# zzzxxxttt/SimpleDepthEstimation

Measured on AMD Instinct MI355X. Metric: training images/sec at 192x640 bs=12/GPU, higher is better.
Workload: dtype bf16; 1 GPU; Supervised ResNet-50 (BASELINE configs[1]), bf16 storage / fp32 accumulate, bs=12/GPU, 192x640, fwd+bwd+optimizer, random-init weights; global_batch=12, parallelism=dp1, hip_graph=True, allreduce_overlap=False

## Files before the change

simpledepthestimation_amd/csrc/conv.hip:

```cpp
#include <type_traits>

#include "common.h"
#include "sde_hip.h"
#include "conv_common.h"

namespace {
using namespace sdeconv;

template <int I> using IC = std::integral_constant<int, I>;

typedef __attribute__((ext_vector_type(4))) float f32x4;
typedef __attribute__((ext_vector_type(8))) __bf16 bf16x8;
typedef __attribute__((ext_vector_type(4))) short s16x4;
typedef __attribute__((ext_vector_type(8))) short s16x8;

template <typename T> struct VecOf;
template <> struct VecOf<float> { static constexpr int V = 4; };
template <> struct VecOf<bf16_t> { static constexpr int V = 8; };
template <> struct VecOf<half_t> { static constexpr int V = 8; };

template <typename T>
__device__ __forceinline__ uint4 gather16(const Gather& g, int n, int ih, int iw, int ci) {
    uint4 z = {0u, 0u, 0u, 0u};
    if (g.reflect) { ih = reflect1(ih, g.IH); iw = reflect1(iw, g.IW); }
// ... 90 lines not shown
    constexpr int CPT = 8 / TPR;
    constexpr int B_ROWS_PER_PASS = NTHREADS / 8;
    constexpr int B_PASSES = (BN + B_ROWS_PER_PASS - 1) / B_ROWS_PER_PASS;
    constexpr int CPAD = 4;
    static_assert(WM * WN == 4, "4 waves");
    extern __shared__ __attribute__((aligned(16))) unsigned char smem[];
    unsigned char* sA = smem;
    unsigned char* sB = smem + 2 * BM * KSTAGE_BYTES;

    const Gather& g = p.g;
    const int tid = threadIdx.x, lane = tid & 63, wave = tid >> 6;
    const int wm = wave / WN, wn = wave % WN;
    const int tiles_n = (p.ldy + BN - 1) / BN;
    const int logical_all = xcd_remap(blockIdx.x, gridDim.x);
    const int tiles_all = gridDim.x / p.ksplit;
    const int split = logical_all / tiles_all, logical = logical_all - split * tiles_all;
    const int tile_m = logical / tiles_n, tile_n = logical - tile_m * tiles_n;
    const int m0 = tile_m * BM, n0 = tile_n * BN;

    const int arow = tid / TPR, ac0 = (tid % TPR) * CPT;
    int an = -1, aih = 0, aiw = 0;
    {
        const int m = m0 + arow;
        if (m < g.M) {
            an = m / (g.OH * g.OW);
            const int rem = m - an * (g.OH * g.OW);
            const int oh = rem / g.OW, ow = rem - oh * g.OW;
            aih = oh * g.stride - g.pad; aiw = ow * g.stride - g.pad;
        }
    }
    const int nk_total = (g.Ktot + BK - 1) / BK;
    const int nk_per = (nk_total + p.ksplit - 1) / p.ksplit;
    const int s_begin = split * nk_per;
    int aci, akh, akw;
    {
        const int k = s_begin * BK + ac0 * V;
        const int tap = k / g.Cin;
        aci = k - tap * g.Cin; akh = tap / g.KW; akw = tap - akh * g.KW;
    }
    const int cc = tid & 7, r0 = tid >> 3;
    const int nk = max(0, min(nk_total, s_begin + nk_per) - s_begin);
    const __amdgpu_buffer_rsrc_t rs0 = make_rsrc(g.x0, (long)g.Bn * g.H0 * g.W0 * g.C0 * (long)sizeof(T));
    const __amdgpu_buffer_rsrc_t rs1 = make_rsrc(g.x1 ? g.x1 : g.x0, g.x1 ? (long)g.Bn * g.IH * g.IW * g.C1 * (long)sizeof(T) : 0);
    const __amdgpu_buffer_rsrc_t rsw = make_rsrc(p.w, (long)p.Cout * g.Ktot * (long)sizeof(T));
    const int mode = src_mode<SRC>(g);
    unsigned rowoff = kOOB;
    if (SRC == SRC_1X1 && an >= 0) rowoff = (unsigned)(((an * g.H0 + aih) * g.W0 + aiw) * g.C0) * (unsigned)sizeof(T);

    const bool kfull = SRC == SRC_1X1 && (g.Ktot % BK) == 0 && !p.no_kfull;
    const bool kfullB = (g.Ktot % BK) == 0 && !p.no_kfull;
    unsigned voffA = kOOB, voffB[B_PASSES];
    if (SRC == SRC_1X1 && an >= 0) voffA = rowoff + (unsigned)(ac0 * V) * (unsigned)sizeof(T);
#pragma unroll
    for (int i = 0; i < B_PASSES; ++i) {
        const int row = r0 + i * B_ROWS_PER_PASS, n = n0 + row;
        voffB[i] = (row < BN && n < p.Cout) ? (unsigned)(n * g.Ktot + cc * V) * (unsigned)sizeof(T) : kOOB;
    }

    uint4 ra[3][CPT], rb[3][B_PASSES];

    auto load_stage = [&](int s, auto SET) {
        constexpr int st = decltype(SET)::value;
        if (SRC == SRC_1X1 && kfull) {
            const unsigned soff = (unsigned)(s_begin + s) * (unsigned)KSTAGE_BYTES;
#pragma unroll
            for (int c = 0; c < CPT; ++c) ra[st][c] = buf_load16s(rs0, voffA + 16u * c, soff);
#pragma unroll
            for (int i = 0; i < B_PASSES; ++i) rb[st][i] = buf_load16s(rsw, voffB[i], soff);
            return;
        }
        if (SRC == SRC_1X1) {
            const int k = (s_begin + s) * BK + ac0 * V;
#pragma unroll
            for (int c = 0; c < CPT; ++c)
                ra[st][c] = buf_load16(rs0, (k + c * V < g.Ktot) ? rowoff + (unsigned)(k + c * V) * (unsigned)sizeof(T) : kOOB);
        } else if (ONE_TAP) {
            unsigned o0, o1;
            gather_off<T, SRC>(g, an >= 0 && akh < g.KH, an, aih + akh, aiw + akw, aci, o0, o1);
#pragma unroll
            for (int c = 0; c < CPT; ++c) {
                uint4 v = buf_load16(rs0, o0 + 16u * c);
                if (mode == SDE_SRC_UPCAT) {
                    const uint4 u = buf_load16(rs1, o1 + 16u * c);
                    v.x |= u.x; v.y |= u.y; v.z |= u.z; v.w |= u.w;
                }
                ra[st][c] = v;
            }
        } else {
            int ci = aci, kh = akh, kw = akw;
#pragma unroll
            for (int c = 0; c < CPT; ++c) {
                unsigned o0, o1;
                gather_off<T, SRC>(g, an >= 0 && kh < g.KH, an, aih + kh, aiw + kw, ci, o0, o1);
                uint4 v = buf_load16(rs0, o0);
                if (mode == SDE_SRC_UPCAT) {
                    const uint4 u = buf_load16(rs1, o1);
                    v.x |= u.x; v.y |= u.y; v.z |= u.z; v.w |= u.w;
                }
                ra[st][c] = v;
                ci += V;
                if (ci == g.Cin) { ci = 0; if (++kw == g.KW) { kw = 0; ++kh; } }
            }
        }
        if (SRC != SRC_1X1) {
            aci += BK;
            while (aci >= g.Cin) { aci -= g.Cin; if (++akw == g.KW) { akw = 0; ++akh; } }
        }
        if (kfullB) {
            const unsigned soff = (unsigned)(s_begin + s) * (unsigned)KSTAGE_BYTES;
#pragma unroll
            for (int i = 0; i < B_PASSES; ++i) rb[st][i] = buf_load16s(rsw, voffB[i], soff);
            return;
        }
        const int k = (s_begin + s) * BK + cc * V;
        const bool kok = k < g.Ktot;
#pragma unroll
        for (int i = 0; i < B_PASSES; ++i) {
            const int row = r0 + i * B_ROWS_PER_PASS;
            const int n = n0 + row;
            constexpr bool rows_fit = B_ROWS_PER_PASS * B_PASSES <= BN;
            const unsigned ow = (kok && (rows_fit || row < BN) && n < p.Cout) ? (unsigned)(n * g.Ktot + k) * (unsigned)sizeof(T) : kOOB;
            rb[st][i] = buf_load16(rsw, ow);
        }
    };
    auto store_stage = [&](int buf, auto SET) {
        constexpr int st = decltype(SET)::value;
#pragma unroll
        for (int c = 0; c < CPT; ++c)
            *reinterpret_cast<uint4*>(sA + (size_t)(buf * BM + arow) * KSTAGE_BYTES + (((ac0 + c) ^ (arow & 7)) << 4)) = ra[st][c];
#pragma unroll
        for (int i = 0; i < B_PASSES; ++i) {
            const int row = r0 + i * B_ROWS_PER_PASS;
            if (B_ROWS_PER_PASS * B_PASSES <= BN || row < BN)
                *reinterpret_cast<uint4*>(sB + (size_t)(buf * BN + row) * KSTAGE_BYTES + ((cc ^ (row & 7)) << 4)) = rb[st][i];
        }
    };

    f32x4 acc[FM][FN];
#pragma unroll
    for (int i = 0; i < FM; ++i)
#pragma unroll
        for (int j = 0; j < FN; ++j) acc[i][j] = f32x4{0.f, 0.f, 0.f, 0.f};

    const int fr = lane & 15, fg = lane >> 4;
    auto compute_stage = [&](int buf) {
#pragma unroll
        for (int kk = 0; kk < 2; ++kk) {
            uint4 a[FM], b[FN];
            const int ch = kk * 4 + fg;
#pragma unroll
            for (int i = 0; i < FM; ++i) {
                const int row = wm * WTM + i * 16 + fr;
                a[i] = *reinterpret_cast<const uint4*>(sA + (size_t)(buf * BM + row) * KSTAGE_BYTES + ((ch ^ (row & 7)) << 4));
            }
#pragma unroll
            for (int j = 0; j < FN; ++j) {
                const int row = wn * WTN + j * 16 + fr;
                b[j] = *reinterpret_cast<const uint4*>(sB + (size_t)(buf * BN + row) * KSTAGE_BYTES + ((ch ^ (row & 7)) << 4));
            }
#pragma unroll
            for (int i = 0; i < FM; ++i)
#pragma unroll
                for (int j = 0; j < FN; ++j) acc[i][j] = mma64<T>(a[i], b[j], acc[i][j]);
        }
    };
    auto step = [&](int st, auto CUR, auto NXT) {
        if (st >= nk) return;
        if (st + 3 < nk) load_stage(st + 3, CUR);
        compute_stage(st & 1);
        if (st + 1 < nk) store_stage((st + 1) & 1, NXT);
        __syncthreads();
    };
    if (nk > 0) load_stage(0, IC<0>{});
    if (nk > 1) load_stage(1, IC<1>{});
    if (nk > 2) load_stage(2, IC<2>{});
    if (nk > 0) store_stage(0, IC<0>{});
    __syncthreads();
    for (int s = 0; s < nk; s += 3) {
        step(s, IC<0>{}, IC<1>{});
        step(s + 1, IC<1>{}, IC<2>{});
        step(s + 2, IC<2>{}, IC<0>{});
    }

    float* sC = reinterpret_cast<float*>(smem);
#pragma unroll
    for (int i = 0; i < FM; ++i)
#pragma unroll
        for (int j = 0; j < FN; ++j)
#pragma unroll
            for (int r = 0; r < 4; ++r) {
                const int row = wm * WTM + i * 16 + fg * 4 + r, col = wn * WTN + j * 16 + fr;
                sC[row * (BN + CPAD) + col] = acc[i][j][r];
            }
    __syncthreads();
    constexpr int G4 = BN / 4;
    const bool vec_ok = (p.ldy % 4) == 0;
    if (p.ksplit > 1) {
        float* wsp = p.ws + (size_t)split * g.M * p.ldy;
        for (int id = tid; id < BM * G4; id += NTHREADS) {
            const int row = id / G4, c0 = (id - row * G4) * 4;
            const int m = m0 + row, n = n0 + c0;
            if (m >= g.M || n >= p.ldy) continue;
            *reinterpret_cast<float4*>(wsp + (size_t)m * p.ldy + n) = *reinterpret_cast<const float4*>(&sC[row * (BN + CPAD) + c0]);
        }
        return;
    }
    for (int id = tid; id < BM * G4; id += NTHREADS) {
        const int row = id / G4, c0 = (id - row * G4) * 4;
        const int m = m0 + row, n = n0 + c0;
        if (m >= g.M || n >= p.ldy) continue;
        const float4 q = *reinterpret_cast<const float4*>(&sC[row * (BN + CPAD) + c0]);
        float v[4] = {q.x, q.y, q.z, q.w};
#pragma unroll
        for (int e = 0; e < 4; ++e) {
            float t = v[e];
            if (p.bias && n + e < p.Cout) t += p.bias[n + e];
            if (p.act == SDE_ACT_ELU) t = t > 0.f ? t : expm1f(t);
            if (n + e >= p.Cout) t = 0.f;
            v[e] = t;
        }
        T* dst = (T*)p.y + (size_t)m * p.ldy + n;
        T o[4];
#pragma unroll
        for (int e = 0; e < 4; ++e) o[e] = from_f32<T>(v[e]);
        if (vec_ok && n + 4 <= p.ldy) {
            if (sizeof(T) == 2) *reinterpret_cast<uint2*>(dst) = *reinterpret_cast<uint2*>(o);
            else *reinterpret_cast<uint4*>(dst) = *reinterpret_cast<uint4*>(o);
        } else {
            for (int e = 0; e < 4 && n + e < p.ldy; ++e) dst[e] = o[e];
        }
        if (p.stats)
            *reinterpret_cast<float4*>(&sC[row * (BN + CPAD) + c0]) = make_float4(to_f32<T>(o[0]), to_f32<T>(o[1]), to_f32<T>(o[2]), to_f32<T>(o[3]));
    }
    if (p.stats) {
        __syncthreads();
        constexpr int PARTS = NTHREADS / BN >= 1 ? NTHREADS / BN : 1;
        float* red = sC + BM * (BN + CPAD);
        const int c = tid % BN, part = tid / BN;
        const int rows = min(BM, g.M - m0);
        float s1 = 0.f, s2 = 0.f;
        if (part < PARTS)
            for (int r = part; r < rows; r += PARTS) { const float t = sC[r * (BN + CPAD) + c]; s1 += t; s2 += t * t; }
        if (part < PARTS) { red[(part * BN + c) * 2] = s1; red[(part * BN + c) * 2 + 1] = s2; }
        __syncthreads();
        if (tid < BN && n0 + tid < p.Cout) {
            float a = 0.f, b = 0.f;
#pragma unroll
            for (int q = 0; q < PARTS; ++q) { a += red[(q * BN + tid) * 2]; b += red[(q * BN + tid) * 2 + 1]; }
            p.stats[((size_t)tile_m * p.Cout + n0 + tid) * 2 + 0] = a;
            p.stats[((size_t)tile_m * p.Cout + n0 + tid) * 2 + 1] = b;
        }
    }
}

template <typename T>
__global__ void __launch_bounds__(256) splitk_finish_kernel(const float* __restrict__ ws, int S, int M, int ldy, int Cout, const float* __restrict__ bias,
                                                            int act, T* __restrict__ y, float* __restrict__ stats) {
    __shared__ float red[16][64][2];
    const int tiles_n = (ldy + 63) / 64;
    const int tile_m = blockIdx.x / tiles_n, tile_n = blockIdx.x - tile_m * tiles_n;
    const int c0 = tile_n * 64 + (threadIdx.x & 15) * 4, rg = threadIdx.x >> 4;
    float s1[4] = {0.f, 0.f, 0.f, 0.f}, s2[4] = {0.f, 0.f, 0.f, 0.f};
    if (c0 < ldy) {
#pragma unroll
        for (int i = 0; i < 4; ++i) {
            const int m = tile_m * 64 + rg + 16 * i;
            if (m >= M) continue;
            float4 a = *reinterpret_cast<const float4*>(ws + (size_t)m * ldy + c0);
            for (int sp = 1; sp < S; ++sp) {
                const float4 b = *reinterpret_cast<const float4*>(ws + ((size_t)sp * M + m) * ldy + c0);
                a.x += b.x; a.y += b.y; a.z += b.z; a.w += b.w;
            }
            float v[4] = {a.x, a.y, a.z, a.w};
            T o[4];
#pragma unroll
            for (int e = 0; e < 4; ++e) {
                float t = v[e];
                if (bias && c0 + e < Cout) t += bias[c0 + e];
                if (act == SDE_ACT_ELU) t = t > 0.f ? t : expm1f(t);
                if (c0 + e >= Cout) t = 0.f;
                o[e] = from_f32<T>(t);
                const float r = to_f32<T>(o[e]);
                s1[e] += r; s2[e] += r * r;
            }
            T* dst = y + (size_t)m * ldy + c0;
            if (sizeof(T) == 2) *reinterpret_cast<uint2*>(dst) = *reinterpret_cast<uint2*>(o);
            else *reinterpret_cast<uint4*>(dst) = *reinterpret_cast<uint4*>(o);
        }
    }
    if (!stats) return;
#pragma unroll
    for (int e = 0; e < 4; ++e) { red[rg][(threadIdx.x & 15) * 4 + e][0] = s1[e]; red[rg][(threadIdx.x & 15) * 4 + e][1] = s2[e]; }
    __syncthreads();
    if (threadIdx.x < 64 && tile_n * 64 + threadIdx.x < Cout) {
        float a = 0.f, b = 0.f;
#pragma unroll
        for (int q = 0; q < 16; ++q) { a += red[q][threadIdx.x][0]; b += red[q][threadIdx.x][1]; }
        stats[((size_t)tile_m * Cout + tile_n * 64 + threadIdx.x) * 2 + 0] = a;
        stats[((size_t)tile_m * Cout + tile_n * 64 + threadIdx.x) * 2 + 1] = b;
    }
}

constexpr int HT_H = 8, HT_W = 16, HALO_W = HT_W + 2, HALO_PIX = (HT_H + 2) * HALO_W;
constexpr int HPIX_STRIDE = 144;
constexpr int HALO_PASSES = (HALO_PIX * 8 + NTHREADS - 1) / NTHREADS;

template <typename T, int SRC>
__device__ __forceinline__ void halo_pix(const Gather& g, bool ok, int n, int ih, int iw, unsigned& p0, unsigned& p1) {
    if (src_reflect<SRC>(g)) { ih = reflect1(ih, g.IH); iw = reflect1(iw, g.IW); ok = ok & ((unsigned)ih < (unsigned)g.IH) & ((unsigned)iw < (unsigned)g.IW); }
    else ok = ok & ((unsigned)ih < (unsigned)g.IH) & ((unsigned)iw < (unsigned)g.IW);
    p1 = kOOB;
    if (src_mode<SRC>(g) == SDE_SRC_UPCAT) {
        p0 = ok ? (unsigned)(((n * g.H0 + (ih >> 1)) * g.W0 + (iw >> 1)) * g.C0) * (unsigned)sizeof(T) : kOOB;
        p1 = (ok && g.C1 > 0) ? (unsigned)(((n * g.IH + ih) * g.IW + iw) * g.C1) * (unsigned)sizeof(T) : kOOB;
    } else {
        p0 = ok ? (unsigned)(((n * g.H0 + ih) * g.W0 + iw) * g.C0) * (unsigned)sizeof(T) : kOOB;
    }
}

template <typename T, int BN, int WM, int WN, int SRC>
__global__ void __launch_bounds__(NTHREADS, 2) halo3_kernel(IGemmP p) {
    constexpr int V = VecOf<T>::V;
    constexpr int BM = HT_H * HT_W;
    constexpr int BK = KSTAGE_BYTES / (int)sizeof(T);
    constexpr int WTM = BM / WM, WTN = BN / WN;
    constexpr int FM = WTM / 16, FN = WTN / 16;
    constexpr int B_ROWS_PER_PASS = NTHREADS / 8;
    constexpr int B_PASSES = (BN + B_ROWS_PER_PASS - 1) / B_ROWS_PER_PASS;
    constexpr int CPAD = 4;
    static_assert(WM * WN == 4 && sizeof(T) == 2, "4 waves, 16-bit storage");
    extern __shared__ __attribute__((aligned(16))) unsigned char smem[];
    unsigned char* sH = smem;
    unsigned char* sB = smem + HALO_PIX * HPIX_STRIDE;

    const Gather& g = p.g;
    const int mode = src_mode<SRC>(g);
    const int tid = threadIdx.x, lane = tid & 63, wave = tid >> 6;
    const int wm = wave / WN, wn = wave % WN;
    const int tiles_n = (p.ldy + BN - 1) / BN, tiles_x = (g.OW + HT_W - 1) / HT_W, tiles_y = (g.OH + HT_H - 1) / HT_H;
    const int logical = xcd_remap(blockIdx.x, gridDim.x);
    const int tile_m = logical / tiles_n, tile_n = logical - tile_m * tiles_n;
    const int img = tile_m / (tiles_x * tiles_y), trem = tile_m - img * (tiles_x * tiles_y);
    const int oy0 = (trem / tiles_x) * HT_H, ox0 = (trem % tiles_x) * HT_W;
    const int n0 = tile_n * BN;
    const __amdgpu_buffer_rsrc_t rs0 = make_rsrc(g.x0, (long)g.Bn * g.H0 * g.W0 * g.C0 * (long)sizeof(T));
    const __amdgpu_buffer_rsrc_t rs1 = make_rsrc(g.x1 ? g.x1 : g.x0, g.x1 ? (long)g.Bn * g.IH * g.IW * g.C1 * (long)sizeof(T) : 0);
    const __amdgpu_buffer_rsrc_t rsw = make_rsrc(p.w, (long)p.Cout * g.Ktot * (long)sizeof(T));

    const int hc = tid & 7;
    unsigned hp0[HALO_PASSES], hp1[HALO_PASSES];
#pragma unroll
    for (int j = 0; j < HALO_PASSES; ++j) {
        const int hp = (tid >> 3) + 32 * j;
        const int hy = hp / HALO_W, hx = hp - hy * HALO_W;
        halo_pix<T, SRC>(g, hp < HALO_PIX, img, oy0 - g.pad + hy, ox0 - g.pad + hx, hp0[j], hp1[j]);
    }
    const int ncb = (g.Cin + BK - 1) / BK;
    const int nst = ncb * 9;
    uint4 rh[HALO_PASSES];
    auto load_halo = [&](int cb) {
        const int ci = cb * BK + hc * V;
#pragma unroll
        for (int j = 0; j < HALO_PASSES; ++j) {
            unsigned o0, o1 = kOOB;
            if (mode == SDE_SRC_UPCAT) {
                o0 = (ci < g.C0 && hp0[j] != kOOB) ? hp0[j] + (unsigned)ci * (unsigned)sizeof(T) : kOOB;
                o1 = (ci >= g.C0 && ci < g.Cin && hp1[j] != kOOB) ? hp1[j] + (unsigned)(ci - g.C0) * (unsigned)sizeof(T) : kOOB;
            } else {
                o0 = (ci < g.Cin && hp0[j] != kOOB) ? hp0[j] + (unsigned)ci * (unsigned)sizeof(T) : kOOB;
            }
            uint4 v = buf_load16(rs0, o0);
            if (mode == SDE_SRC_UPCAT) {
                const uint4 u = buf_load16(rs1, o1);
                v.x |= u.x; v.y |= u.y; v.z |= u.z; v.w |= u.w;
            }
            rh[j] = v;
        }
    };
    auto store_halo = [&]() {
#pragma unroll
        for (int j = 0; j < HALO_PASSES; ++j) {
            const int hp = (tid >> 3) + 32 * j;
            if (hp < HALO_PIX) *reinterpret_cast<uint4*>(sH + hp * HPIX_STRIDE + hc * 16) = rh[j];
        }
    };
    const int cc = tid & 7, r0 = tid >> 3;
    uint4 rb[3][B_PASSES];
    auto load_b = [&](int s, auto SET) {
        constexpr int st = decltype(SET)::value;
        const int cb = s / 9, tap = s - cb * 9;
        const int ci = cb * BK + cc * V;
        const int k = tap * g.Cin + ci;
#pragma unroll
        for (int i = 0; i < B_PASSES; ++i) {
            const int row = r0 + i * B_ROWS_PER_PASS, n = n0 + row;
            rb[st][i] = buf_load16(rsw, (ci < g.Cin && row < BN && n < p.Cout) ? (unsigned)(n * g.Ktot + k) * (unsigned)sizeof(T) : kOOB);
        }
    };
    auto store_b = [&](int buf, auto SET) {
        constexpr int st = decltype(SET)::value;
#pragma unroll
        for (int i = 0; i < B_PASSES; ++i) {
            const int row = r0 + i * B_ROWS_PER_PASS;
            if (B_ROWS_PER_PASS * B_PASSES <= BN || row < BN)
                *reinterpret_cast<uint4*>(sB + (size_t)(buf * BN + row) * KSTAGE_BYTES + ((cc ^ (row & 7)) << 4)) = rb[st][i];
        }
    };

    f32x4 acc[FM][FN];
#pragma unroll
    for (int i = 0; i < FM; ++i)
#pragma unroll
        for (int j = 0; j < FN; ++j) acc[i][j] = f32x4{0.f, 0.f, 0.f, 0.f};

    const int fr = lane & 15, fg = lane >> 4;
    int abase[FM];
#pragma unroll
    for (int i = 0; i < FM; ++i) abase[i] = ((wm * FM + i) * HALO_W + fr) * HPIX_STRIDE + fg * 16;
    auto compute_stage = [&](int buf, int tap) {
        const int toff = ((tap / 3) * HALO_W + (tap % 3)) * HPIX_STRIDE;
#pragma unroll
        for (int kk = 0; kk < 2; ++kk) {
            uint4 a[FM], b[FN];
#pragma unroll
            for (int i = 0; i < FM; ++i) a[i] = *reinterpret_cast<const uint4*>(sH + abase[i] + toff + kk * 64);
#pragma unroll
            for (int j = 0; j < FN; ++j) {
                const int row = wn * WTN + j * 16 + fr;
                b[j] = *reinterpret_cast<const uint4*>(sB + (size_t)(buf * BN + row) * KSTAGE_BYTES + (((kk * 4 + fg) ^ (row & 7)) << 4));
            }
#pragma unroll
            for (int i = 0; i < FM; ++i)
#pragma unroll
                for (int j = 0; j < FN; ++j) acc[i][j] = mma64<T>(a[i], b[j], acc[i][j]);
        }
    };
    auto step = [&](int st, auto CUR, auto NXT) {
        if (st >= nst) return;
        const int cb = st / 9, tap = st - cb * 9;
        if (st + 3 < nst) load_b(st + 3, CUR);
        if (tap == 0 && cb + 1 < ncb) load_halo(cb + 1);
        compute_stage(st & 1, tap);
        if (st + 1 < nst) store_b((st + 1) & 1, NXT);
        __syncthreads();
        if (tap == 8 && cb + 1 < ncb) {
            store_halo();
            __syncthreads();
        }
    };
    load_halo(0);
    load_b(0, IC<0>{});
    if (nst > 1) load_b(1, IC<1>{});
    if (nst > 2) load_b(2, IC<2>{});
    store_halo();
    store_b(0, IC<0>{});
    __syncthreads();
    for (int s = 0; s < nst; s += 3) {
        step(s, IC<0>{}, IC<1>{});
        step(s + 1, IC<1>{}, IC<2>{});
        step(s + 2, IC<2>{}, IC<0>{});
    }

    float* sC = reinterpret_cast<float*>(smem);
#pragma unroll
    for (int i = 0; i < FM; ++i)
#pragma unroll
        for (int j = 0; j < FN; ++j)
#pragma unroll
            for (int r = 0; r < 4; ++r) {
                const int row = wm * WTM + i * 16 + fg * 4 + r, col = wn * WTN + j * 16 + fr;
                sC[row * (BN + CPAD) + col] = acc[i][j][r];
            }
    __syncthreads();
    constexpr int G4 = BN / 4;
    const bool vec_ok = (p.ldy % 4) == 0;
    if (p.bn_y) {
        static_assert(NTHREADS % G4 == 0, "a thread keeps one channel group");
        const int c0 = (tid % G4) * 4, n = n0 + c0;
        const float4 mean = *reinterpret_cast<const float4*>(p.bnp + n), rstd = *reinterpret_cast<const float4*>(p.bnp + p.Cout + n);
        const float4 scl = *reinterpret_cast<const float4*>(p.bnp + 2 * p.Cout + n), shf = *reinterpret_cast<const float4*>(p.bnp + 3 * p.Cout + n);
        const float mn[4] = {mean.x, mean.y, mean.z, mean.w}, rs[4] = {rstd.x, rstd.y, rstd.z, rstd.w};
        const float sc[4] = {scl.x, scl.y, scl.z, scl.w}, sf[4] = {shf.x, shf.y, shf.z, shf.w};
        float a1[4] = {0.f, 0.f, 0.f, 0.f}, a2[4] = {0.f, 0.f, 0.f, 0.f};
        for (int id = tid; id < BM * G4; id += NTHREADS) {
            const int row = id / G4;
            const int oy = oy0 + row / HT_W, ox = ox0 + row % HT_W;
            if (!(oy < g.OH && ox < g.OW)) continue;
            const size_t off = ((size_t)(img * g.OH + oy) * g.OW + ox) * p.ldy + n;
            const uint2 yr = *reinterpret_cast<const uint2*>((const T*)p.bn_y + off);
            const T* yt = reinterpret_cast<const T*>(&yr);
            const float4 q = *reinterpret_cast<const float4*>(&sC[row * (BN + CPAD) + c0]);
            const float v[4] = {q.x, q.y, q.z, q.w};
            T o[4];
            if (p.bn_gb) {
                const uint2 gr = *reinterpret_cast<const uint2*>((const T*)p.bn_gb + off), orr = *reinterpret_cast<const uint2*>((const T*)p.bn_out + off);
                const T* gt = reinterpret_cast<const T*>(&gr);
                const T* ot = reinterpret_cast<const T*>(&orr);
#pragma unroll
                for (int e = 0; e < 4; ++e) {
                    const float yv = to_f32<T>(yt[e]);
                    const float ga = to_f32<T>(from_f32<T>(v[e]));
                    o[e] = from_f32<T>(to_f32<T>(ot[e]) > 0.f ? ga + to_f32<T>(gt[e]) : 0.f);
                    const float t = to_f32<T>(o[e]);
                    a1[e] += t; a2[e] += t * ((yv - mn[e]) * rs[e]);
                }
            } else {
#pragma unroll
            for (int e = 0; e < 4; ++e) {
                const float yv = to_f32<T>(yt[e]);
                o[e] = from_f32<T>(fmaf(yv, sc[e], sf[e]) > 0.f ? v[e] : 0.f);
                const float t = to_f32<T>(o[e]);
                a1[e] += t; a2[e] += t * ((yv - mn[e]) * rs[e]);
            }
            }
            *reinterpret_cast<uint2*>((T*)p.y + off) = *reinterpret_cast<uint2*>(o);
        }
        __syncthreads();
        constexpr int PARTS = NTHREADS / G4;
        float* red = sC;
        const int part = tid / G4;
#pragma unroll
        for (int e = 0; e < 4; ++e) { red[(part * BN + c0 + e) * 2] = a1[e]; red[(part * BN + c0 + e) * 2 + 1] = a2[e]; }
        __syncthreads();
        if (tid < BN && n0 + tid < p.Cout) {
            float a = 0.f, b = 0.f;
#pragma unroll
            for (int q = 0; q < PARTS; ++q) { a += red[(q * BN + tid) * 2]; b += red[(q * BN + tid) * 2 + 1]; }
            p.stats[((size_t)tile_m * p.Cout + n0 + tid) * 2 + 0] = a;
            p.stats[((size_t)tile_m * p.Cout + n0 + tid) * 2 + 1] = b;
        }
        return;
    }
    for (int id = tid; id < BM * G4; id += NTHREADS) {
        const int row = id / G4, c0 = (id - row * G4) * 4;
        const int oy = oy0 + row / HT_W, ox = ox0 + row % HT_W, n = n0 + c0;
        const bool rok = oy < g.OH && ox < g.OW;
        if (!rok || n >= p.ldy) {
            if (p.stats && !rok) *reinterpret_cast<float4*>(&sC[row * (BN + CPAD) + c0]) = make_float4(0.f, 0.f, 0.f, 0.f);
            continue;
        }
        const float4 q = *reinterpret_cast<const float4*>(&sC[row * (BN + CPAD) + c0]);
        float v[4] = {q.x, q.y, q.z, q.w};
#pragma unroll
        for (int e = 0; e < 4; ++e) {
            float t = v[e];
            if (p.bias && n + e < p.Cout) t += p.bias[n + e];
            if (p.act == SDE_ACT_ELU) t = t > 0.f ? t : expm1f(t);
            if (n + e >= p.Cout) t = 0.f;
            v[e] = t;
        }
        T* dst = (T*)p.y + ((size_t)(img * g.OH + oy) * g.OW + ox) * p.ldy + n;
        T o[4];
#pragma unroll
        for (int e = 0; e < 4; ++e) o[e] = from_f32<T>(v[e]);
        if (vec_ok && n + 4 <= p.ldy) *reinterpret_cast<uint2*>(dst) = *reinterpret_cast<uint2*>(o);
        else for (int e = 0; e < 4 && n + e < p.ldy; ++e) dst[e] = o[e];
        if (p.stats)
            *reinterpret_cast<float4*>(&sC[row * (BN + CPAD) + c0]) = make_float4(to_f32<T>(o[0]), to_f32<T>(o[1]), to_f32<T>(o[2]), to_f32<T>(o[3]));
    }
    if (p.stats) {
        __syncthreads();
        constexpr int PARTS = NTHREADS / BN >= 1 ? NTHREADS / BN : 1;
        float* red = sC + BM * (BN + CPAD);
        const int c = tid % BN, part = tid / BN;
        float s1 = 0.f, s2 = 0.f;
        if (part < PARTS)
            for (int r = part; r < BM; r += PARTS) { const float t = sC[r * (BN + CPAD) + c]; s1 += t; s2 += t * t; }
        if (part < PARTS) { red[(part * BN + c) * 2] = s1; red[(part * BN + c) * 2 + 1] = s2; }
        __syncthreads();
        if (tid < BN && n0 + tid < p.Cout) {
            float a = 0.f, b = 0.f;
#pragma unroll
            for (int q = 0; q < PARTS; ++q) { a += red[(q * BN + tid) * 2]; b += red[(q * BN + tid) * 2 + 1]; }
            p.stats[((size_t)tile_m * p.Cout + n0 + tid) * 2 + 0] = a;
            p.stats[((size_t)tile_m * p.Cout + n0 + tid) * 2 + 1] = b;
        }
    }
}

struct WGradP {
    Gather g;
    const void* dy;
    float* slab;
    int Cout, ldd, rows_per_split;
    int single_buf;
};

template <typename T> struct WGTraits;
template <> struct WGTraits<bf16_t> { static constexpr int BR = 64; };
template <> struct WGTraits<half_t> { static constexpr int BR = 64; };
template <> struct WGTraits<float> { static constexpr int BR = 32; };

template <typename T> struct TrRead;
template <> struct TrRead<bf16_t> {
    static __device__ __forceinline__ uint4 rd(const unsigned char* tile, int stride, int p0, int col0, int lane) {
        const int g = lane >> 4, i = lane & 15, q = i >> 2, pp = i & 3;
        const int row = p0 + 8 * g + q;
        const unsigned char* a0 = tile + (size_t)row * stride + (size_t)((((col0 + 4 * pp) * 2)) ^ ((row & 8) << 4));
#if defined(SDE_WGRAD_SAFE_READ)
        const int col = col0 + i;
        s16x8 v;
#pragma unroll
        for (int j = 0; j < 8; ++j) v[j] = *reinterpret_cast<const short*>(tile + (size_t)(p0 + 8 * g + j) * stride + (size_t)((col * 2) ^ (((p0 + 8 * g + j) & 8) << 4)));
        (void)a0;
        return __builtin_bit_cast(uint4, v);
#else
        typedef __attribute__((address_space(3))) s16x4 lds_s16x4;
        const s16x4 lo = __builtin_amdgcn_ds_read_tr16_b64_v4i16((lds_s16x4*)(a0));
        const s16x4 hi = __builtin_amdgcn_ds_read_tr16_b64_v4i16((lds_s16x4*)(a0 + 4 * (size_t)stride));
        s16x8 v = {lo[0], lo[1], lo[2], lo[3], hi[0], hi[1], hi[2], hi[3]};
        return __builtin_bit_cast(uint4, v);
#endif
    }
};
template <> struct TrRead<half_t> : TrRead<bf16_t> {};
template <> struct TrRead<float> {
    static __device__ __forceinline__ uint4 rd(const unsigned char* tile, int stride, int p0, int col0, int lane) {
        const int g = lane >> 4, i = lane & 15;
        const unsigned char* a = tile + (size_t)(p0 + 4 * g) * stride + (size_t)(col0 + i) * 4;
        uint4 v;
        v.x = *reinterpret_cast<const uint32_t*>(a);
        v.y = *reinterpret_cast<const uint32_t*>(a + stride);
        v.z = *reinterpret_cast<const uint32_t*>(a + 2 * (size_t)stride);
        v.w = *reinterpret_cast<const uint32_t*>(a + 3 * (size_t)stride);
        return v;
    }
};

template <typename T, int BMG, int BNG, int WM, int WN, int SRC, bool ONE_TAP>
__global__ void __launch_bounds__(NTHREADS, (BMG <= 64 && sizeof(T) == 2) ? 3 : 2) wgrad_kernel(WGradP p) {
    constexpr int V = VecOf<T>::V;
    constexpr int BR = WGTraits<T>::BR;
    constexpr int SUBP = 64 / (int)sizeof(T);
    constexpr int NSUB = BR / SUBP;
    constexpr int WTM = BMG / WM, WTN = BNG / WN;
    constexpr int FM = WTM / 16, FN = WTN / 16;
    constexpr int STRA = sizeof(T) == 2 ? 288 : BMG * (int)sizeof(T) + 16;
    constexpr int STRB = sizeof(T) == 2 ? 288 : BNG * (int)sizeof(T) + 16;
    constexpr int SWZ = sizeof(T) == 2 ? 1 : 0;
    static_assert(sizeof(T) != 2 || (BMG <= 128 && BNG <= 128), "bf16 rows must fit the 288-byte stride with the half swap");
    constexpr int ACH = BMG / V, BCH = BNG / V;
    constexpr int TPP = NTHREADS / BR;
    constexpr int CPTB = BCH / TPP;
    constexpr int CPTA = (ACH + TPP - 1) / TPP;
    static_assert(WM * WN == 4, "4 waves");
    static_assert(BCH % TPP == 0, "B tile chunking");
    extern __shared__ __attribute__((aligned(16))) unsigned char smem[];
    unsigned char* sA = smem;
    unsigned char* sB = smem + (p.single_buf ? 1 : 2) * BR * STRA;

    const Gather& g = p.g;
    const int tid = threadIdx.x, lane = tid & 63, wave = tid >> 6;
    const int wm = wave / WN, wn = wave % WN;
    const int tiles_co = (p.Cout + BMG - 1) / BMG, tiles_k = (g.Ktot + BNG - 1) / BNG;
    const int logical = xcd_remap(blockIdx.x, gridDim.x);
    const int split = logical / (tiles_co * tiles_k), rem_t = logical - split * (tiles_co * tiles_k);
    const int co0 = (rem_t % tiles_co) * BMG, k0 = (rem_t / tiles_co) * BNG;
    const int mbeg = split * p.rows_per_split, mend = min(g.M, mbeg + p.rows_per_split);

    const int px = tid / TPP, tq = tid % TPP;
    int bkh[CPTB], bkw[CPTB], bci[CPTB];
#pragma unroll
    for (int c = 0; c < CPTB; ++c) {
        const int k = k0 + (tq * CPTB + c) * V;
        if (k < g.Ktot) {
            const int tap = k / g.Cin;
            bci[c] = k - tap * g.Cin; bkh[c] = tap / g.KW; bkw[c] = tap - bkh[c] * g.KW;
        } else {
            bci[c] = -1; bkh[c] = 0; bkw[c] = 0;
        }
    }
    int pn, poh, pow_;
    {
        const int m = mbeg + px;
        pn = m / (g.OH * g.OW);
        const int rem = m - pn * (g.OH * g.OW);
        poh = rem / g.OW; pow_ = rem - poh * g.OW;
    }
    const __amdgpu_buffer_rsrc_t rs0 = make_rsrc(g.x0, (long)g.Bn * g.H0 * g.W0 * g.C0 * (long)sizeof(T));
    const __amdgpu_buffer_rsrc_t rs1 = make_rsrc(g.x1 ? g.x1 : g.x0, g.x1 ? (long)g.Bn * g.IH * g.IW * g.C1 * (long)sizeof(T) : 0);
    const __amdgpu_buffer_rsrc_t rsd = make_rsrc(p.dy, (long)g.M * p.ldd * (long)sizeof(T));
    const int mode = src_mode<SRC>(g);
    uint4 ra[3][CPTA], rb[3][CPTB];
    auto load_stage = [&](int s, auto SET) {
        constexpr int st = decltype(SET)::value;
        const int m = mbeg + s * BR + px;
        const bool mok = m < mend;
#pragma unroll
        for (int c = 0; c < CPTA; ++c) {
            const int ch = tq * CPTA + c;
            const int co = co0 + ch * V;
            const unsigned od = (mok && ch < ACH && co < p.ldd) ? (unsigned)(m * p.ldd + co) * (unsigned)sizeof(T) : kOOB;
            ra[st][c] = buf_load16(rsd, od);
        }
        const int ih0 = poh * g.stride - g.pad, iw0 = pow_ * g.stride - g.pad;
        if (SRC == SRC_1X1) {
            const unsigned rowoff = (unsigned)(((pn * g.H0 + ih0) * g.W0 + iw0) * g.C0) * (unsigned)sizeof(T);
#pragma unroll
            for (int c = 0; c < CPTB; ++c)
                rb[st][c] = buf_load16(rs0, (mok && bci[c] >= 0) ? rowoff + (unsigned)bci[c] * (unsigned)sizeof(T) : kOOB);
        } else if (ONE_TAP) {
            unsigned o0, o1;
            gather_off<T, SRC>(g, mok && bci[0] >= 0, pn, ih0 + bkh[0], iw0 + bkw[0], bci[0], o0, o1);
#pragma unroll
            for (int c = 0; c < CPTB; ++c) {
                uint4 v = buf_load16(rs0, o0 + 16u * c);
                if (mode == SDE_SRC_UPCAT) {
                    const uint4 u = buf_load16(rs1, o1 + 16u * c);
                    v.x |= u.x; v.y |= u.y; v.z |= u.z; v.w |= u.w;
                }
                rb[st][c] = v;
            }
        } else {
#pragma unroll
            for (int c = 0; c < CPTB; ++c) {
                unsigned o0, o1;
                gather_off<T, SRC>(g, mok && bci[c] >= 0, pn, ih0 + bkh[c], iw0 + bkw[c], bci[c], o0, o1);
                uint4 v = buf_load16(rs0, o0);
                if (mode == SDE_SRC_UPCAT) {
                    const uint4 u = buf_load16(rs1, o1);
                    v.x |= u.x; v.y |= u.y; v.z |= u.z; v.w |= u.w;
                }
                rb[st][c] = v;
            }
        }
        pow_ += BR;
        while (pow_ >= g.OW) { pow_ -= g.OW; if (++poh == g.OH) { poh = 0; ++pn; } }
    };
    auto store_stage = [&](int buf, auto SET) {
        constexpr int st = decltype(SET)::value;
#pragma unroll
        for (int c = 0; c < CPTA; ++c) {
            const int ch = tq * CPTA + c;
            if (ch < ACH) *reinterpret_cast<uint4*>(sA + (size_t)(buf * BR + px) * STRA + ((ch * 16) ^ (SWZ * ((px & 8) << 4)))) = ra[st][c];
        }
#pragma unroll
        for (int c = 0; c < CPTB; ++c)
            *reinterpret_cast<uint4*>(sB + (size_t)(buf * BR + px) * STRB + (((tq * CPTB + c) * 16) ^ (SWZ * ((px & 8) << 4)))) = rb[st][c];
    };

    f32x4 acc[FM][FN];
#pragma unroll
    for (int i = 0; i < FM; ++i)
#pragma unroll
        for (int j = 0; j < FN; ++j) acc[i][j] = f32x4{0.f, 0.f, 0.f, 0.f};

    const int ns = (mend - mbeg + BR - 1) / BR;
    auto compute_stage = [&](int buf) {
        const unsigned char* tA = sA + (size_t)buf * BR * STRA;
        const unsigned char* tB = sB + (size_t)buf * BR * STRB;
#pragma unroll
        for (int kk = 0; kk < NSUB; ++kk) {
            uint4 a[FM], b[FN];
#pragma unroll
            for (int i = 0; i < FM; ++i) a[i] = TrRead<T>::rd(tA, STRA, kk * SUBP, wm * WTM + i * 16, lane);
#pragma unroll
            for (int j = 0; j < FN; ++j) b[j] = TrRead<T>::rd(tB, STRB, kk * SUBP, wn * WTN + j * 16, lane);
#pragma unroll
            for (int i = 0; i < FM; ++i)
#pragma unroll
                for (int j = 0; j < FN; ++j) acc[i][j] = mma64<T>(a[i], b[j], acc[i][j]);
        }
    };
    const int dbl = p.single_buf ? 0 : 1;
// ... 914 lines not shown
```

Baseline: 1929 images/s.

## Unroll halo 3x3 conv loop per channel block with compile-time taps and padded halo stride

Restructures the halo 3x3 implicit-GEMM main loop into per-channel-block groups of nine compile-time taps, removing runtime divisions and branch checks per stage. The next halo load now starts at tap 3 instead of tap 0, which shortens how long its registers stay live. The halo pixel stride in LDS grows from 144 to 160 bytes, presumably to change the bank-conflict pattern of A-fragment reads at the cost of more shared memory. Full unrolling enlarges the code and may raise register pressure.

After: 1952 images/s, median of 6. 1.01x the previous value.

```diff
diff --git a/simpledepthestimation_amd/csrc/conv.hip b/simpledepthestimation_amd/csrc/conv.hip
--- a/simpledepthestimation_amd/csrc/conv.hip
+++ b/simpledepthestimation_amd/csrc/conv.hip
@@ -416,7 +416,7 @@
 }
 
 constexpr int HT_H = 8, HT_W = 16, HALO_W = HT_W + 2, HALO_PIX = (HT_H + 2) * HALO_W;
-constexpr int HPIX_STRIDE = 144;
+constexpr int HPIX_STRIDE = 160;
 constexpr int HALO_PASSES = (HALO_PIX * 8 + NTHREADS - 1) / NTHREADS;
 
 template <typename T, int SRC>
@@ -470,7 +470,6 @@
         halo_pix<T, SRC>(g, hp < HALO_PIX, img, oy0 - g.pad + hy, ox0 - g.pad + hx, hp0[j], hp1[j]);
     }
     const int ncb = (g.Cin + BK - 1) / BK;
-    const int nst = ncb * 9;
     uint4 rh[HALO_PASSES];
     auto load_halo = [&](int cb) {
         const int ci = cb * BK + hc * V;
@@ -500,9 +499,8 @@
     };
     const int cc = tid & 7, r0 = tid >> 3;
     uint4 rb[3][B_PASSES];
-    auto load_b = [&](int s, auto SET) {
+    auto load_b = [&](int cb, int tap, auto SET) {
         constexpr int st = decltype(SET)::value;
-        const int cb = s / 9, tap = s - cb * 9;
         const int ci = cb * BK + cc * V;
         const int k = tap * g.Cin + ci;
 #pragma unroll
@@ -549,31 +547,35 @@
                 for (int j = 0; j < FN; ++j) acc[i][j] = mma64<T>(a[i], b[j], acc[i][j]);
         }
     };
-    auto step = [&](int st, auto CUR, auto NXT) {
-        if (st >= nst) return;
-        const int cb = st / 9, tap = st - cb * 9;
-        if (st + 3 < nst) load_b(st + 3, CUR);
-        if (tap == 0 && cb + 1 < ncb) load_halo(cb + 1);
-        compute_stage(st & 1, tap);
-        if (st + 1 < nst) store_b((st + 1) & 1, NXT);
+    constexpr int HALO_TAP = 3;
+    auto stage = [&](int cb, auto TAP, auto LAST) {
+        constexpr int tap = decltype(TAP)::value;
+        constexpr bool last = decltype(LAST)::value;
+        if constexpr (tap + 3 < 9) load_b(cb, tap + 3, IC<tap % 3>{});
+        else if constexpr (!last) load_b(cb + 1, tap + 3 - 9, IC<tap % 3>{});
+        if constexpr (tap == HALO_TAP && !last) load_halo(cb + 1);
+        compute_stage((cb + tap) & 1, tap);
+        if constexpr (tap < 8 || !last) store_b((cb + tap + 1) & 1, IC<(tap + 1) % 3>{});
         __syncthreads();
-        if (tap == 8 && cb + 1 < ncb) {
+        if constexpr (tap == 8 && !last) {
             store_halo();
             __syncthreads();
         }
     };
+    auto block = [&](int cb, auto LAST) {
+        stage(cb, IC<0>{}, LAST); stage(cb, IC<1>{}, LAST); stage(cb, IC<2>{}, LAST);
+        stage(cb, IC<3>{}, LAST); stage(cb, IC<4>{}, LAST); stage(cb, IC<5>{}, LAST);
+        stage(cb, IC<6>{}, LAST); stage(cb, IC<7>{}, LAST); stage(cb, IC<8>{}, LAST);
+    };
     load_halo(0);
-    load_b(0, IC<0>{});
-    if (nst > 1) load_b(1, IC<1>{});
-    if (nst > 2) load_b(2, IC<2>{});
+    load_b(0, 0, IC<0>{});
+    load_b(0, 1, IC<1>{});
+    load_b(0, 2, IC<2>{});
     store_halo();
     store_b(0, IC<0>{});
     __syncthreads();
-    for (int s = 0; s < nst; s += 3) {
-        step(s, IC<0>{}, IC<1>{});
-        step(s + 1, IC<1>{}, IC<2>{});
-        step(s + 2, IC<2>{}, IC<0>{});
-    }
+    for (int cb = 0; cb + 1 < ncb; ++cb) block(cb, std::false_type{});
+    block(ncb - 1, std::true_type{});
 
     float* sC = reinterpret_cast<float*>(smem);
 #pragma unroll
```
